# broadinstitute/Tangram

Measured on NVIDIA H100. Metric: map_cells_to_space iterations/sec, higher is better.
Workload: dtype bf16 operands / f32 accumulate+state

## Files before the change

### tangram_b200/csrc/gemm_tc.cuh

```cuda
#pragma once
#include <cuda.h>
#include <cstdio>
#include "common.cuh"
#include "gemm_simt.cuh"

namespace tgb {

constexpr int TC_BM = 128;
constexpr int TC_BK = 64;
constexpr int TC_MMA_K = 16;
constexpr int TC_BN = 256;
constexpr int TC_THREADS = 384;
constexpr int TC_ACC = TC_BN / 2;

__device__ __forceinline__ uint32_t smem_u32(const void* p) { return (uint32_t)__cvta_generic_to_shared(p); }

__device__ __forceinline__ void mbar_init(uint64_t* bar, uint32_t count) {
  asm volatile("mbarrier.init.shared::cta.b64 [%0], %1;" ::"r"(smem_u32(bar)), "r"(count));
}
__device__ __forceinline__ void mbar_expect_tx(uint64_t* bar, uint32_t bytes) {
  asm volatile("mbarrier.arrive.expect_tx.shared::cta.b64 _, [%0], %1;" ::"r"(smem_u32(bar)), "r"(bytes) : "memory");
}
__device__ __forceinline__ void mbar_wait(uint64_t* bar, uint32_t parity) {
  asm volatile(
      "{\n\t.reg .pred p;\n\t"
      "WAIT_LOOP:\n\t"
      "mbarrier.try_wait.parity.shared::cta.b64 p, [%0], %1;\n\t"
      "@p bra WAIT_DONE;\n\t"
      "bra WAIT_LOOP;\n\t"
      "WAIT_DONE:\n\t}"
      ::"r"(smem_u32(bar)), "r"(parity) : "memory");
}
__device__ __forceinline__ void mbar_arrive(uint64_t* bar) {
  asm volatile("mbarrier.arrive.shared::cta.b64 _, [%0];" ::"r"(smem_u32(bar)) : "memory");
}
__device__ __forceinline__ void fence_barrier_init() { asm volatile("fence.mbarrier_init.release.cluster;" ::: "memory"); }
__device__ __forceinline__ void mbar_arrive_cluster(uint64_t* bar, uint32_t cta) {
  asm volatile(
      "{\n\t.reg .b32 ra;\n\t"
      "mapa.shared::cluster.u32 ra, %0, %1;\n\t"
      "mbarrier.arrive.shared::cluster.b64 _, [ra];\n\t}"
      ::"r"(smem_u32(bar)), "r"(cta) : "memory");
}
__device__ __forceinline__ int cluster_rank() { uint32_t r; asm volatile("mov.u32 %0, %%cluster_ctarank;" : "=r"(r)); return (int)r; }
__device__ __forceinline__ int cluster_index() { uint32_t r; asm volatile("mov.u32 %0, %%clusterid.x;" : "=r"(r)); return (int)r; }
__device__ __forceinline__ int cluster_count() { uint32_t r; asm volatile("mov.u32 %0, %%nclusterid.x;" : "=r"(r)); return (int)r; }
__device__ __forceinline__ void cluster_sync() {
  asm volatile("barrier.cluster.arrive.release;\n\tbarrier.cluster.wait.acquire;" ::: "memory");
}

constexpr uint64_t kPolicyEvictNormal = 0x1000000000000000ull;
constexpr uint64_t kPolicyEvictLast = 0x14F0000000000000ull;
constexpr uint64_t kPolicyEvictFirst = 0x12F0000000000000ull;
__device__ __forceinline__ void prefetch_l2(const void* p) { asm volatile("prefetch.global.L2 [%0];" ::"l"(p)); }
__device__ __forceinline__ void tma_load_2d(const CUtensorMap* map, uint64_t* bar, void* dst, int c0, int c1, uint64_t policy) {
  asm volatile(
      "cp.async.bulk.tensor.2d.shared::cluster.global.tile.mbarrier::complete_tx::bytes.L2::cache_hint [%0], [%1, {%3, %4}], [%2], %5;"
      ::"r"(smem_u32(dst)), "l"(map), "r"(smem_u32(bar)), "r"(c0), "r"(c1), "l"(policy) : "memory");
}
__device__ __forceinline__ void tma_load_2d_pair(const CUtensorMap* map, uint64_t* bar, void* dst, int c0, int c1, uint64_t policy) {
  asm volatile(
      "cp.async.bulk.tensor.2d.shared::cluster.global.tile.mbarrier::complete_tx::bytes.multicast::cluster.L2::cache_hint"
      " [%0], [%1, {%3, %4}], [%2], %5, %6;"
      ::"r"(smem_u32(dst)), "l"(map), "r"(smem_u32(bar)), "r"(c0), "r"(c1), "h"((uint16_t)0x3), "l"(policy) : "memory");
}
__device__ __forceinline__ void tma_prefetch_desc(const CUtensorMap* map) {
  asm volatile("prefetch.tensormap [%0];" ::"l"(map) : "memory");
}
__device__ __forceinline__ void tma_store_2d(const CUtensorMap* map, const void* src, int c0, int c1, uint64_t policy) {
  asm volatile(
      "cp.async.bulk.tensor.2d.global.shared::cta.bulk_group.L2::cache_hint [%0, {%2, %3}], [%1], %4;"
      ::"l"(map), "r"(smem_u32(src)), "r"(c0), "r"(c1), "l"(policy) : "memory");
}
__device__ __forceinline__ void bulk_commit() { asm volatile("cp.async.bulk.commit_group;" ::: "memory"); }
__device__ __forceinline__ void bulk_wait_read_all() { asm volatile("cp.async.bulk.wait_group.read 0;" ::: "memory"); }
__device__ __forceinline__ void fence_proxy_async_smem() { asm volatile("fence.proxy.async.shared::cta;" ::: "memory"); }
template <int ID>
__device__ __forceinline__ void named_bar_sync(int threads) {
  asm volatile("bar.sync %0, %1;" ::"n"(ID), "r"(threads) : "memory");
}
__device__ __forceinline__ void ldmatrix_x4(uint32_t addr, uint32_t (&r)[4]) {
  asm volatile("ldmatrix.sync.aligned.m8n8.x4.shared.b16 {%0, %1, %2, %3}, [%4];"
               : "=r"(r[0]), "=r"(r[1]), "=r"(r[2]), "=r"(r[3]) : "r"(addr) : "memory");
}
__device__ __forceinline__ void stmatrix_x4(uint32_t addr, const uint32_t (&r)[4]) {
  asm volatile("stmatrix.sync.aligned.m8n8.x4.shared.b16 [%0], {%1, %2, %3, %4};"
               ::"r"(addr), "r"(r[0]), "r"(r[1]), "r"(r[2]), "r"(r[3]) : "memory");
}

__device__ __forceinline__ void setmaxnreg_producer() { asm volatile("setmaxnreg.dec.sync.aligned.u32 40;"); }
__device__ __forceinline__ void setmaxnreg_consumer() { asm volatile("setmaxnreg.inc.sync.aligned.u32 232;"); }

__device__ __forceinline__ void wgmma_fence() { asm volatile("wgmma.fence.sync.aligned;" ::: "memory"); }
__device__ __forceinline__ void wgmma_commit() { asm volatile("wgmma.commit_group.sync.aligned;" ::: "memory"); }
template <int N>
__device__ __forceinline__ void wgmma_wait() { asm volatile("wgmma.wait_group.sync.aligned %0;" ::"n"(N) : "memory"); }
__device__ __forceinline__ void acc_fence(float (&d)[TC_ACC]) {
// ... 24 lines not shown
        "+f"(d[40]), "+f"(d[41]), "+f"(d[42]), "+f"(d[43]), "+f"(d[44]), "+f"(d[45]), "+f"(d[46]), "+f"(d[47]),
        "+f"(d[48]), "+f"(d[49]), "+f"(d[50]), "+f"(d[51]), "+f"(d[52]), "+f"(d[53]), "+f"(d[54]), "+f"(d[55]),
        "+f"(d[56]), "+f"(d[57]), "+f"(d[58]), "+f"(d[59]), "+f"(d[60]), "+f"(d[61]), "+f"(d[62]), "+f"(d[63]),
        "+f"(d[64]), "+f"(d[65]), "+f"(d[66]), "+f"(d[67]), "+f"(d[68]), "+f"(d[69]), "+f"(d[70]), "+f"(d[71]),
        "+f"(d[72]), "+f"(d[73]), "+f"(d[74]), "+f"(d[75]), "+f"(d[76]), "+f"(d[77]), "+f"(d[78]), "+f"(d[79]),
        "+f"(d[80]), "+f"(d[81]), "+f"(d[82]), "+f"(d[83]), "+f"(d[84]), "+f"(d[85]), "+f"(d[86]), "+f"(d[87]),
        "+f"(d[88]), "+f"(d[89]), "+f"(d[90]), "+f"(d[91]), "+f"(d[92]), "+f"(d[93]), "+f"(d[94]), "+f"(d[95]),
        "+f"(d[96]), "+f"(d[97]), "+f"(d[98]), "+f"(d[99]), "+f"(d[100]), "+f"(d[101]), "+f"(d[102]), "+f"(d[103]),
        "+f"(d[104]), "+f"(d[105]), "+f"(d[106]), "+f"(d[107]), "+f"(d[108]), "+f"(d[109]), "+f"(d[110]), "+f"(d[111]),
        "+f"(d[112]), "+f"(d[113]), "+f"(d[114]), "+f"(d[115]), "+f"(d[116]), "+f"(d[117]), "+f"(d[118]), "+f"(d[119]),
        "+f"(d[120]), "+f"(d[121]), "+f"(d[122]), "+f"(d[123]), "+f"(d[124]), "+f"(d[125]), "+f"(d[126]), "+f"(d[127])
      : "l"(a_desc), "l"(b_desc), "r"(accumulate), "n"(TA), "n"(TB));
}
__device__ __forceinline__ uint64_t make_smem_desc(uint32_t saddr, uint32_t lbo_bytes, uint32_t sbo_bytes) {
  uint64_t d = 0;
  d |= (uint64_t)((saddr & 0x3FFFF) >> 4);
  d |= (uint64_t)((lbo_bytes >> 4) & 0x3FFF) << 16;
  d |= (uint64_t)((sbo_bytes >> 4) & 0x3FFF) << 32;
  d |= (uint64_t)1 << 62;
  return d;
}

template <bool KMAJOR, int ROWS>
struct OperandTile {
  static constexpr int kBytes = ROWS * TC_BK * 2;
  static __device__ __forceinline__ void load(const CUtensorMap* map, uint64_t* bar, uint8_t* dst, int mn0, int k0, uint64_t policy) {
    if (KMAJOR) {
      tma_load_2d(map, bar, dst, k0, mn0, policy);
    } else {
#pragma unroll
      for (int b = 0; b < ROWS / 64; ++b) tma_load_2d(map, bar, dst + b * 8192, mn0 + b * 64, k0, policy);
    }
  }
  static __device__ __forceinline__ void load_half_pair(const CUtensorMap* map, uint64_t* bar, uint8_t* dst, int mn0, int k0, int h,
                                                        uint64_t policy) {
    constexpr int HALF = ROWS / 2;
    if (KMAJOR) {
      tma_load_2d_pair(map, bar, dst + h * HALF * 128, k0, mn0 + h * HALF, policy);
    } else {
#pragma unroll
      for (int b = 0; b < HALF / 64; ++b)
        tma_load_2d_pair(map, bar, dst + h * HALF * 128 + b * 8192, mn0 + h * HALF + b * 64, k0, policy);
    }
  }
  static __device__ __forceinline__ uint64_t desc(uint32_t saddr, int k_step ) {
    if (KMAJOR) return make_smem_desc(saddr + k_step * (TC_MMA_K * 2), 16, 1024);
    return make_smem_desc(saddr + k_step * (TC_MMA_K * 128), 8192, 1024);
  }
};

struct EpiSmem {
  uint8_t* buf;
  uint64_t* full;
  uint64_t* free;
  uint32_t parity;
};
__device__ __forceinline__ void tile_mn(int w, int tiles_m, int tiles_n, int group_m, int& m, int& n) {
  const int per_group = group_m * tiles_n;
  const int g = w / per_group, r = w - g * per_group;
  const int rows = min(group_m, tiles_m - g * group_m);
  n = r / rows;
  m = g * group_m + (r - n * rows);
}
struct TileCoord {
  int m0, n0;
  int tile_n;
  int tiles_n;
  int split;
};

__device__ __forceinline__ float quad_sum(float v) {
  v += __shfl_xor_sync(0xffffffffu, v, 1);
  v += __shfl_xor_sync(0xffffffffu, v, 2);
  return v;
}

struct TcEpiStore {
  static constexpr int kSmemBytes = 0;
  float* C; int ldc; size_t split_stride; int M;
  int accumulate;
  __device__ __forceinline__ void prologue(const TileCoord&, int) const {}
  __device__ __forceinline__ void load(int, int, const EpiSmem&) const {}
  __device__ __forceinline__ void run(const float (&d)[TC_ACC], const TileCoord& t, int row, int lane, int, const EpiSmem&) const {
    float* base = C + (size_t)t.split * split_stride;
#pragma unroll
    for (int h = 0; h < 2; ++h) {
      const int r = row + 8 * h;
      if (r >= M) continue;
#pragma unroll
      for (int j = 0; j < TC_BN / 8; ++j) {
        const int col = t.n0 + 8 * j + 2 * (lane & 3);
        if (col < ldc) {
          float2* dst = reinterpret_cast<float2*>(base + (size_t)r * ldc + col);
          float2 v = make_float2(d[4 * j + 2 * h], d[4 * j + 2 * h + 1]);
          if (accumulate) { const float2 o = *dst; v.x += o.x; v.y += o.y; }
          *dst = v;
        }
      }
    }
  }
};

struct TcEpiDpStore {
  static constexpr int kSmemBytes = TC_BM * TC_BN * 2;
  static constexpr int kHalfBytes = kSmemBytes / 2;
  static constexpr int kBoxBytes = 64 * 128;
  CUtensorMap pt_map, dq_map;
  int ld;
  const float* center;
  float* rpart;
  int M;
  __device__ __forceinline__ int boxes(int r0, int n0) const { return r0 < M ? min(TC_BN / 64, (ld - n0) / 64) : 0; }
  __device__ __forceinline__ void prologue(const TileCoord&, int) const {}
  __device__ __forceinline__ void load(int m0, int n0, const EpiSmem& es) const {
#pragma unroll
    for (int h = 0; h < 2; ++h) {
      mbar_wait(&es.free[h], es.parity ^ 1);
      const int nb = boxes(m0 + 64 * h, n0);
      mbar_expect_tx(&es.full[h], nb * kBoxBytes);
      for (int b = 0; b < nb; ++b)
        tma_load_2d(&pt_map, &es.full[h], es.buf + h * kHalfBytes + b * kBoxBytes, n0 + 64 * b, m0 + 64 * h, kPolicyEvictFirst);
    }
  }
  __device__ __forceinline__ void run(const float (&d)[TC_ACC], const TileCoord& t, int row, int lane, int cw,
                                      const EpiSmem& es) const {
    const int r0 = t.m0 + 64 * cw;
    const int nb = boxes(r0, t.n0);
    float c[2];
#pragma unroll
// ... 66 lines not shown
      float* drow = dp + (size_t)r * ld;
      float racc = 0.f;
#pragma unroll
      for (int j = 0; j < TC_BN / 8; ++j) {
        const int col = t.n0 + 8 * j + 2 * (lane & 3);
        if (live && col < ld) {
          const __nv_bfloat162 h2 = *reinterpret_cast<const __nv_bfloat162*>(prow + col);
          const __nv_bfloat162 m2 = *reinterpret_cast<const __nv_bfloat162*>(prow + plane + col);
          const __nv_bfloat162 l2 = *reinterpret_cast<const __nv_bfloat162*>(prow + 2 * plane + col);
          const float p0 = (__low2float(l2) + __low2float(m2)) + __low2float(h2);
          const float p1 = (__high2float(l2) + __high2float(m2)) + __high2float(h2);
          const float v0 = d[4 * j + 2 * h], v1 = d[4 * j + 2 * h + 1];
          racc = fmaf(p0, v0, racc);
          racc = fmaf(p1, v1, racc);
          *reinterpret_cast<float2*>(drow + col) = make_float2(v0, v1);
        }
      }
      racc = quad_sum(racc);
      if (live && (lane & 3) == 0) rpart[(size_t)t.tile_n * M + r] = racc;
    }
  }
};

struct __align__(16) RowConst { float lse, r, h, pad; };

__device__ __forceinline__ float fast_ex2(float x) { float y; asm("ex2.approx.ftz.f32 %0, %1;" : "=f"(y) : "f"(x)); return y; }
__device__ __forceinline__ float fast_rcp(float x) { float y; asm("rcp.approx.ftz.f32 %0, %1;" : "=f"(y) : "f"(x)); return y; }
__device__ __forceinline__ float fast_sqrt(float x) { float y; asm("sqrt.approx.ftz.f32 %0, %1;" : "=f"(y) : "f"(x)); return y; }

struct TcMaps { CUtensorMap m[3]; };
__device__ __constant__ int kPairA[6] = {2, 0, 1, 1, 0, 0};
__device__ __constant__ int kPairB[6] = {0, 2, 1, 0, 1, 0};

template <bool A_KMAJOR, bool B_KMAJOR, int STAGES, class Epi>
__global__ void __launch_bounds__(TC_THREADS, 1)
k_gemm_tc(const __grid_constant__ TcMaps maps_a, const __grid_constant__ TcMaps maps_b, int n_pairs,
          int k_total, int k_per_split, int tiles_m, int tiles_n, int splits, int group_m, uint64_t policy_a,
          uint64_t policy_b, int tm_off, int k_off, const __grid_constant__ Epi epi) {
  using TileA = OperandTile<A_KMAJOR, TC_BM>;
  using TileB = OperandTile<B_KMAJOR, TC_BN>;
  constexpr int kStageBytes = TileA::kBytes + TileB::kBytes;
  constexpr int kTA = A_KMAJOR ? 0 : 1, kTB = B_KMAJOR ? 0 : 1;
  constexpr uint32_t kConsumerWarps = 8;

  extern __shared__ uint8_t smem_raw[];
  uint8_t* smem = reinterpret_cast<uint8_t*>(((uintptr_t)smem_raw + 1023) & ~(uintptr_t)1023);
  __shared__ __align__(8) uint64_t full_bar[STAGES];
  __shared__ __align__(8) uint64_t empty_bar[STAGES];
  __shared__ __align__(8) uint64_t epi_full[2], epi_free[2];

  const int wg = threadIdx.x >> 7, lane = threadIdx.x & 31;
  const int tiles_mp = (tiles_m + 1) / 2;
  const int total = tiles_mp * tiles_n * splits;
  EpiSmem es{smem + STAGES * kStageBytes, epi_full, epi_free, 0};

  if (threadIdx.x == 0) {
    tma_prefetch_desc(&maps_a.m[0]);
    tma_prefetch_desc(&maps_b.m[0]);
#pragma unroll
    for (int s = 0; s < STAGES; ++s) { mbar_init(&full_bar[s], 1); mbar_init(&empty_bar[s], 2 * kConsumerWarps); }
    if constexpr (Epi::kSmemBytes > 0) {
      for (int h = 0; h < 2; ++h) { mbar_init(&epi_full[h], 1); mbar_init(&epi_free[h], 1); }
    }
    fence_barrier_init();
  }
  cluster_sync();

  if (wg == 0) {
    setmaxnreg_producer();
    if (threadIdx.x == 0) {
      uint32_t kbg = 0;
      for (int w = cluster_index(); w < total; w += cluster_count()) {
        const int z = w / (tiles_n * tiles_mp);
        int tp_i, tn_i;
        tile_mn(w - z * tiles_n * tiles_mp, tiles_mp, tiles_n, group_m, tp_i, tn_i);
        const int tm_i = 2 * tp_i + cluster_rank();
        const bool live = tm_i < tiles_m;
        const int n0 = tn_i * TC_BN, m0 = (tm_off + tm_i) * TC_BM;
        const int k_begin = k_off + z * k_per_split;
        const int k_end = min(k_total, k_begin + k_per_split);
        const int num_kb = (k_end - k_begin + TC_BK - 1) / TC_BK;
        for (int pr = 6 - n_pairs; pr < 6; ++pr) {
          const CUtensorMap* ma = &maps_a.m[kPairA[pr]];
          const CUtensorMap* mb = &maps_b.m[kPairB[pr]];
#pragma unroll 1
          for (int kb = 0; kb < num_kb; ++kb, ++kbg) {
            const int s = kbg % STAGES;
            const uint32_t ph = (kbg / STAGES) & 1;
            mbar_wait(&empty_bar[s], ph ^ 1);
            uint8_t* sa = smem + s * kStageBytes;
            uint8_t* sb = sa + TileA::kBytes;
            mbar_expect_tx(&full_bar[s], live ? kStageBytes : TileB::kBytes);
            const int k0 = k_begin + kb * TC_BK;
            if (live) TileA::load(ma, &full_bar[s], sa, m0, k0, policy_a);
            TileB::load_half_pair(mb, &full_bar[s], sb, n0, k0, cluster_rank(), policy_b);
#ifndef TGB_SKIP_EPI
            if (Epi::kSmemBytes > 0 && live && pr == 6 - n_pairs && kb + 1 == min(STAGES, num_kb)) epi.load(m0, n0, es);
#endif
          }
        }
        if (live) es.parity ^= 1;
      }
    }
  } else {
    setmaxnreg_consumer();
    const int cw = wg - 1;
    const int ct = threadIdx.x - 128;
    const int row_in_tile = 64 * cw + 16 * ((threadIdx.x >> 5) & 3) + (lane >> 2);
    float acc[TC_ACC];
#pragma unroll
    for (int i = 0; i < TC_ACC; ++i) acc[i] = 0.f;
    uint32_t kbg = 0;
    for (int w = cluster_index(); w < total; w += cluster_count()) {
      TileCoord t;
      t.split = w / (tiles_n * tiles_mp);
      int tp_i;
      tile_mn(w - t.split * tiles_n * tiles_mp, tiles_mp, tiles_n, group_m, tp_i, t.tile_n);
      t.tiles_n = tiles_n;
      t.n0 = t.tile_n * TC_BN;
      t.m0 = (tm_off + 2 * tp_i + cluster_rank()) * TC_BM;
      const bool live = t.m0 < (tm_off + tiles_m) * TC_BM;
      const int k_begin = k_off + t.split * k_per_split;
      const int k_end = min(k_total, k_begin + k_per_split);
      const int total_kb = (k_end - k_begin + TC_BK - 1) / TC_BK * n_pairs;
#ifndef TGB_SKIP_EPI
      if (live) epi.prologue(t, ct);
#endif
      acc_fence(acc);
      for (int kb = 0; kb < total_kb; ++kb, ++kbg) {
        const int s = kbg % STAGES;
        const uint32_t ph = (kbg / STAGES) & 1;
        mbar_wait(&full_bar[s], ph);
        const uint32_t sa = smem_u32(smem + s * kStageBytes) + cw * 8192;
        const uint32_t sb = smem_u32(smem + s * kStageBytes) + TileA::kBytes;
        wgmma_fence();
#pragma unroll
        for (int k = 0; k < TC_BK / TC_MMA_K; ++k)
          wgmma_m64n256k16<kTA, kTB>(acc, TileA::desc(sa, k), TileB::desc(sb, k), (kb > 0 || k > 0) ? 1u : 0u);
        wgmma_commit();
        wgmma_wait<1>();
        if (kb > 0 && lane < 2) mbar_arrive_cluster(&empty_bar[(kbg - 1) % STAGES], lane);
      }
      wgmma_wait<0>();
      acc_fence(acc);
      if (total_kb > 0 && lane < 2) mbar_arrive_cluster(&empty_bar[(kbg - 1) % STAGES], lane);
#ifndef TGB_SKIP_EPI
      if (t.m0 < (tm_off + tiles_m) * TC_BM) {
        epi.run(acc, t, t.m0 + row_in_tile, lane, cw, es);
        es.parity ^= 1;
      }
#endif
    }
  }
  cluster_sync();
}

typedef CUresult (*PFN_encodeTiled)(CUtensorMap*, CUtensorMapDataType, cuuint32_t, void*, const cuuint64_t*,
                                    const cuuint64_t*, const cuuint32_t*, const cuuint32_t*, CUtensorMapInterleave,
                                    CUtensorMapSwizzle, CUtensorMapL2promotion, CUtensorMapFloatOOBfill);

struct TcContext {
  PFN_encodeTiled encode = nullptr;
  int num_sms = 132;
  const void* smem_fn[16] = {};
  int smem_bytes[16] = {};
  int clusters[16] = {};
};

static inline int tc_init(TcContext& tc, char* err, size_t n) {
  void* fn = nullptr;
  cudaDriverEntryPointQueryResult qres;
  cudaError_t e = cudaGetDriverEntryPoint("cuTensorMapEncodeTiled", &fn, cudaEnableDefault, &qres);
  if (e != cudaSuccess || fn == nullptr || qres != cudaDriverEntryPointSuccess) {
    snprintf(err, n, "cuTensorMapEncodeTiled not available from the driver (%s)", cudaGetErrorString(e));
    return -2;
  }
  tc.encode = (PFN_encodeTiled)fn;
  int dev = 0;
  cudaGetDevice(&dev);
  cudaDeviceGetAttribute(&tc.num_sms, cudaDevAttrMultiProcessorCount, dev);
  return 0;
}

static inline int tc_make_map(TcContext& tc, CUtensorMap* map, const void* base, uint64_t cols, uint64_t rows,
                              uint64_t ld, uint32_t box_inner, uint32_t box_outer, char* err, size_t n) {
  cuuint64_t dims[2] = {cols, rows};
  cuuint64_t strides[1] = {ld * 2};
  cuuint32_t box[2] = {box_inner, box_outer};
  cuuint32_t estr[2] = {1, 1};
  CUresult r = tc.encode(map, CU_TENSOR_MAP_DATA_TYPE_BFLOAT16, 2, const_cast<void*>(base), dims, strides, box, estr,
                         CU_TENSOR_MAP_INTERLEAVE_NONE, CU_TENSOR_MAP_SWIZZLE_128B, CU_TENSOR_MAP_L2_PROMOTION_L2_256B,
                         CU_TENSOR_MAP_FLOAT_OOB_FILL_NONE);
  if (r != CUDA_SUCCESS) {
    snprintf(err, n, "cuTensorMapEncodeTiled failed (%d) cols=%llu rows=%llu ld=%llu box=%ux%u", (int)r,
             (unsigned long long)cols, (unsigned long long)rows, (unsigned long long)ld, box_inner, box_outer);
    return -2;
  }
  return 0;
}

template <class Kern, class... Args>
static inline int tc_launch(TcContext& tc, Kern kern, int smem, long long pairs, int keep_sms, cudaStream_t s, const char* name,
                            char* err, size_t n, Args... args) {
  cudaLaunchAttribute attr[1];
  attr[0].id = cudaLaunchAttributeClusterDimension;
  attr[0].val.clusterDim.x = 2;
  attr[0].val.clusterDim.y = 1;
  attr[0].val.clusterDim.z = 1;
  cudaLaunchConfig_t cfg = {};
  cfg.blockDim = dim3(TC_THREADS);
  cfg.dynamicSmemBytes = (size_t)smem;
  cfg.stream = s;
  cfg.attrs = attr;
  cfg.numAttrs = 1;
  const void* key = reinterpret_cast<const void*>(kern);
  int slot = -1;
  for (int i = 0; i < 16; ++i) {
    if (tc.smem_fn[i] == key) { slot = i; break; }
    if (tc.smem_fn[i] == nullptr && slot < 0) slot = i;
  }
  if (slot < 0) { snprintf(err, n, "launch %s: more than 16 tensor-core kernels", name); return -2; }
  if (tc.smem_fn[slot] != key || tc.smem_bytes[slot] != smem) {
    cudaError_t e = cudaFuncSetAttribute(kern, cudaFuncAttributeMaxDynamicSharedMemorySize, smem);
    if (e != cudaSuccess) { snprintf(err, n, "cudaFuncSetAttribute(smem=%d): %s", smem, cudaGetErrorString(e)); return -2; }
    cfg.gridDim = dim3(2);
    int c = 0;
    e = cudaOccupancyMaxActiveClusters(&c, kern, &cfg);
    if (e != cudaSuccess || c < 1) {
      snprintf(err, n, "launch %s: no 2-CTA cluster with %d B of shared memory fits (%s)", name, smem, cudaGetErrorString(e));
      return -2;
    }
    tc.smem_fn[slot] = key; tc.smem_bytes[slot] = smem; tc.clusters[slot] = c;
  }
  const int clusters = std::max(1, tc.clusters[slot] - (keep_sms + 1) / 2);
  cfg.gridDim = dim3((unsigned)(2 * (pairs < clusters ? pairs : clusters)));
  cudaError_t e = cudaLaunchKernelEx(&cfg, kern, args...);
  if (e == cudaSuccess) e = cudaGetLastError();
  if (e != cudaSuccess) { snprintf(err, n, "launch %s: %s", name, cudaGetErrorString(e)); return -2; }
  return 0;
}

constexpr int TC_STAGE_BYTES = (TC_BM + TC_BN) * TC_BK * 2;
constexpr int TC_SMEM_LIMIT = 227 * 1024;
template <class Epi>
constexpr int tc_stages() {
  const int fit = (TC_SMEM_LIMIT - 2048 - Epi::kSmemBytes) / TC_STAGE_BYTES;
  return fit < 4 ? fit : 4;
}
template <class Epi>
constexpr int tc_smem() { return tc_stages<Epi>() * TC_STAGE_BYTES + Epi::kSmemBytes + 1024; }
constexpr int TC_SMEM = tc_smem<TcEpiStore>();
static inline int tc_dp_row_parts(int V) { return (int)ceil_div(V, TC_BN); }
static inline int tc_splits(int num_sms, long long tiles, long long k_total, int min_k) {
  long long s = (2LL * num_sms + tiles - 1) / tiles;
  const long long max_s = (k_total + min_k - 1) / min_k;
  if (s > max_s) s = max_s;
  if (s < 1) s = 1;
  const long long kps = ((k_total + s - 1) / s + TC_BK - 1) / TC_BK * TC_BK;
  return (int)((k_total + kps - 1) / kps);
}
static inline int tc_splits_for_chain(long long k_total, int max_chain) {
  long long s = (k_total + max_chain - 1) / max_chain;
  if (s < 1) s = 1;
  const long long kps = ((k_total + s - 1) / s + TC_BK - 1) / TC_BK * TC_BK;
  return (int)((k_total + kps - 1) / kps);
}
static inline int tc_forward_splits(int num_sms, int N, int V, int Ke) {
  return tc_splits(num_sms, (long long)ceil_div(V, TC_BM) * ceil_div(Ke, TC_BN), N, 512);
}
static inline int tc_kps(int k_total, int splits) {
  return (int)(round_up(ceil_div(k_total, splits), TC_BK));
}
static inline long long tc_pairs(int tiles_m, int tiles_n, int splits) { return (long long)(tiles_m + 1) / 2 * tiles_n * splits; }

static inline int tc_make_maps(TcContext& tc, TcMaps* maps, const __nv_bfloat16* base, size_t plane_elems, int n_planes,
                               uint64_t cols, uint64_t rows, uint64_t ld, uint32_t bi, uint32_t bo, char* err, size_t n) {
  for (int p = 0; p < 3; ++p) {
    const __nv_bfloat16* ptr = base + (size_t)(p < n_planes ? p : 0) * plane_elems;
    if (tc_make_map(tc, &maps->m[p], ptr, cols, rows, ld, bi, bo, err, n)) return -2;
  }
  return 0;
}

struct TcPlan {
  TcMaps a, b;
  CUtensorMap pt, dq;
  bool ready = false;
};

static inline int tc_forward_plan(TcContext& tc, TcPlan& pl, const __nv_bfloat16* P, size_t p_plane, const __nv_bfloat16* Sx,
                                  size_t s_plane, int planes, int N, int V, int Ke, int ld, char* err, size_t n) {
  if (tc_make_maps(tc, &pl.a, P, p_plane, planes, V, N, ld, 64, 64, err, n)) return -2;
  if (tc_make_maps(tc, &pl.b, Sx, s_plane, planes, Ke, N, Ke, 64, 64, err, n)) return -2;
  pl.ready = true;
  return 0;
}
static inline int tc_forward_launch(TcContext& tc, const TcPlan& pl, int n_pairs, float* out, int N, int V, int Ke, int splits,
                                    cudaStream_t s, char* err, size_t n) {
  auto kern = k_gemm_tc<false, false, tc_stages<TcEpiStore>(), TcEpiStore>;
  TcEpiStore epi{out, Ke, (size_t)V * Ke, V, 0};
  const int tm = (int)ceil_div(V, TC_BM), tn = (int)ceil_div(Ke, TC_BN);
  return tc_launch(tc, kern, TC_SMEM, tc_pairs(tm, tn, splits), 0, s, "tc_gemm_fwd", err, n, pl.a, pl.b, n_pairs, N, tc_kps(N, splits),
                   tm, tn, splits, 1, kPolicyEvictNormal, kPolicyEvictNormal, 0, 0, epi);
}
static inline int tc_forward_launch_rows(TcContext& tc, const TcPlan& pl, int n_pairs, float* out, int accumulate, int row0, int row1,
                                         int V, int Ke, int keep_sms, cudaStream_t s, char* err, size_t n) {
  auto kern = k_gemm_tc<false, false, tc_stages<TcEpiStore>(), TcEpiStore>;
  TcEpiStore epi{out, Ke, (size_t)V * Ke, V, accumulate};
  const int tm = (int)ceil_div(V, TC_BM), tn = (int)ceil_div(Ke, TC_BN);
  return tc_launch(tc, kern, TC_SMEM, tc_pairs(tm, tn, 1), keep_sms, s, "tc_gemm_fwd", err, n, pl.a, pl.b, n_pairs, row1,
                   (int)round_up(row1 - row0, TC_BK), tm, tn, 1, 1, kPolicyEvictNormal, kPolicyEvictNormal, 0, row0, epi);
}

static inline int tc_dpstore_plan(TcContext& tc, TcPlan& pl, const __nv_bfloat16* Sxb, size_t s_plane, const __nv_bfloat16* dYb,
                                  size_t dy_plane, int planes, int N, int V, int Ke, char* err, size_t n) {
  if (tc_make_maps(tc, &pl.a, Sxb, s_plane, planes, Ke, N, Ke, 64, TC_BM, err, n)) return -2;
  if (tc_make_maps(tc, &pl.b, dYb, dy_plane, planes, Ke, V, Ke, 64, TC_BN / 2, err, n)) return -2;
  pl.ready = true;
  return 0;
}
static inline int tc_dpstore_epi_plan(TcContext& tc, TcPlan& pl, const __nv_bfloat16* Pt, const __nv_bfloat16* dq, int N, int ld,
                                      char* err, size_t n) {
  if (tc_make_map(tc, &pl.pt, Pt, ld, N, ld, 64, 64, err, n)) return -2;
  return tc_make_map(tc, &pl.dq, dq, ld, N, ld, 64, 64, err, n);
}
template <class Epi>
static inline int tc_dpstore_launch(TcContext& tc, const TcPlan& pl, int n_pairs, const Epi& epi, int row0, int row1, int V, int Ke,
                                    int keep_sms, cudaStream_t s, char* err, size_t n) {
  const int tn = (int)ceil_div(V, TC_BN);
  auto kern = k_gemm_tc<true, true, tc_stages<Epi>(), Epi>;
  constexpr int smem = tc_smem<Epi>();
  const int tm0 = row0 / TC_BM, tm = (int)ceil_div(row1, TC_BM) - tm0;
  return tc_launch(tc, kern, smem, tc_pairs(tm, tn, 1), keep_sms, s, "tc_gemm_bwd_dp", err, n, pl.a, pl.b, n_pairs, Ke, Ke, tm, tn, 1, 1,
                   kPolicyEvictNormal, kPolicyEvictLast, tm0, 0, epi);
}

}
```

### tangram_b200/csrc/tangram_b200.cu

```cuda
#include "../../include/tangram_b200.h"

#include <algorithm>
#include <cmath>
#include <cstdarg>
#include <cstdio>
#include <cstdlib>
#include <cstring>
#include <mutex>
#include <string>
#include <thread>
#include <vector>

#include "common.cuh"
#include "kernels_elem.cuh"
#include "gemm_simt.cuh"
#include "gemm_tc.cuh"
#include "adam_rows.cuh"
#include "legacy_rng.cuh"
#include "agreement.cuh"
#include "annotate.cuh"
#include "project.cuh"
#include "group_stats.cuh"
#include "neighbors.cuh"
#include "mt19937_jump.h"
// ... 1990 lines not shown
      if (nr) CK(cudaMemcpy(out_host, d.p, nr * sizeof(float), cudaMemcpyDefault));
      if (hp.n) CK(cudaMemcpy(out_host + nr, hp.p, hp.n * sizeof(float), cudaMemcpyDefault));
    }
    return TGB200_OK;
  };
  if (nm == "Y") { src = h->Y.p; cnt = vk; }
  else if (nm == "M") return state(h->M, h->Mh);
  else if (nm == "v") return state(h->v, h->vh);
  else if (nm == "m") return h->bf16 ? state(h->mb, h->mbh) : state(h->m, h->mh);
  else if (nm == "Pb" && h->x3) return widened(h->Pb.p, nv, 3);
  else if (nm == "Pf" && !h->tcm) { src = h->Pf.p; cnt = nv; }
  else if (nm == "dpf" && h->x3) { src = h->dpf.p; cnt = nv; }
  else if (nm == "stats") { src = reinterpret_cast<const float*>(h->stats.p); cnt = (int64_t)h->N * 4; }
  else if (nm == "rowc" && h->bf16) { src = reinterpret_cast<const float*>(h->rowc.p); cnt = (int64_t)h->N * 4; }
  else if (nm == "zsum" && h->bf16) { src = h->zsum.p; cnt = h->N; }
  else if (nm == "inv_zt" && h->bf16) { src = h->inv_zt.p; cnt = h->N; }
  else if (nm == "lseA" && h->bf16) { src = h->lseA; cnt = h->N; }
  else if (nm == "lseT" && h->bf16) { src = h->lseT; cnt = h->N; }
  else if (nm == "pxsum" && h->pxsum.p) { src = h->pxsum.p; cnt = h->N; }
  else if (nm == "l1sum" && h->l1sum.p) { src = h->l1sum.p; cnt = h->N; }
  else if (nm == "l2sum" && h->l2sum.p) { src = h->l2sum.p; cnt = h->N; }
  else if (nm == "dY") {
    src = h->dY.p; cnt = vk;
    if (h->tcm && out_host) {
      if (cap < cnt) return fail(TGB200_ERR_INVALID, "buffer 'dY' needs %lld floats", (long long)cnt);
      CKS(widen_bf16(h->dYb.p, vk, h->x3 ? 3 : 1, out_host));
      *n = cnt;
      return TGB200_OK;
    }
  }
  else if ((nm == "dq" || nm == "Pb") && h->bf16) return widened(nm == "dq" ? h->dq.p : h->Pb.p, nv, 1);
  else if (nm == "rcenter" && h->bf16) { src = h->rcenter.p; cnt = h->N; }
  else if (nm == "rdot") { src = h->rdot.p; cnt = h->N; }
  else if (nm == "ngc") { src = h->ngc.p; cnt = h->K; }
  else if (nm == "ngr") { src = h->ngr.p; cnt = h->V; }
  else if (nm == "nwg" && h->nwg.p) { src = h->nwg.p; cnt = h->K; }
  else if (nm == "nag" && h->nag.p) { src = h->nag.p; cnt = h->K; }
  else if (nm == "Sx") { src = h->Sx.p; cnt = (int64_t)h->N * h->Ke; }
  else if (nm == "tail") { src = h->Y.p + vk; cnt = kTail; }
  else if (h->constrained && (nm == "F" || nm == "f" || nm == "mF" || nm == "vF")) {
    src = nm == "F" ? h->Fl.p : nm == "f" ? h->fsig.p : nm == "mF" ? h->mF.p : h->vF.p;
    cnt = h->N;
  }
  else if (nm == "Sf" && h->constrained) { src = h->Sf.p; cnt = (int64_t)h->N * h->Ke; }
  else if (nm == "fscal" && h->constrained) { src = h->fscal.p; cnt = 2; }
  else if (nm == "shape") {
    *n = 5;
    if (!out_host) return TGB200_OK;
    if (cap < 5) return fail(TGB200_ERR_INVALID, "cap < 5");
    out_host[0] = (float)h->Ke; out_host[1] = (float)h->ld; out_host[2] = (float)h->fwd_splits; out_host[3] = (float)h->r_parts;
    out_host[4] = (float)h->nchunks;
    return TGB200_OK;
  } else if (nm == "ring") {
    *n = 1;
    if (!out_host) return TGB200_OK;
    if (cap < 1) return fail(TGB200_ERR_INVALID, "cap < 1");
    out_host[0] = (float)h->ring_rows;
    return TGB200_OK;
  } else if (nm == "legacy_init") {
    *n = 8;
    if (!out_host) return TGB200_OK;
    if (cap < 8) return fail(TGB200_ERR_INVALID, "cap < 8");
    for (int i = 0; i < 8; ++i) out_host[i] = h->legacy_stats[i];
    return TGB200_OK;
  } else return fail(TGB200_ERR_INVALID, "unknown debug buffer '%s'", name);
  *n = cnt;
// ... 674 lines not shown
}

extern "C" int tgb200_group_stats(const float* X, int64_t x_ld, const int64_t* indptr, const int32_t* indices,
                                  const float* data, int64_t nnz, int64_t rows, int64_t n_genes,
                                  const int32_t* labels, int32_t n_labels, double* sum_out, double* sumsq_out,
                                  int64_t* nnz_out, int64_t block_rows, int32_t device, void* stream) {
  return group_stats_pass(GsValue::kIdentity, 1.0, X, x_ld, indptr, indices, data, nnz, rows, n_genes, labels, n_labels,
                          sum_out, sumsq_out, nnz_out, block_rows, device, stream);
}

extern "C" int tgb200_group_stats_expm1(const float* X, int64_t x_ld, const int64_t* indptr, const int32_t* indices,
                                        const float* data, int64_t nnz, int64_t rows, int64_t n_genes,
                                        const int32_t* labels, int32_t n_labels, double* sum_out, double* sumsq_out,
                                        int64_t* nnz_out, int64_t block_rows, int32_t device, void* stream,
                                        double scale) {
  if (!std::isfinite(scale)) return fail(TGB200_ERR_INVALID, "scale=%g is not finite", scale);
  return group_stats_pass(GsValue::kExpm1, scale, X, x_ld, indptr, indices, data, nnz, rows, n_genes, labels, n_labels,
                          sum_out, sumsq_out, nnz_out, block_rows, device, stream);
}

#ifdef TGB_OVERLAP_PROBE
extern "C" TGB200_API int tgb200_debug_overlap_probe(tgb200_mapper* h, int32_t kind, int32_t cap, int32_t update_ctas,
                                                     int32_t what, int32_t reps, float* out) {
  if (!h || !out || reps < 1 || what < 1 || what > 3) return fail(TGB200_ERR_INVALID, "bad argument");
  if (!h->bf16 || !h->pipelined || h->host_state || !h->plan_dp.ready || !h->plan_fwd.ready)
    return fail(TGB200_ERR_STATE, "needs a resident, pipelined bf16 handle that has run an iteration");
  CK(cudaSetDevice(h->cfg.device));
  const int c0 = h->chunk_row[0], c1 = h->chunk_row[1], c2 = h->chunk_row[2];
  const AdamScalars a = adam_scalars(h->cfg, h->step > 0 ? h->step : 1, 0.1f);
  const AdamRowsArgs ar{h->M.p, h->mb.p, h->v.p, h->dq.p, h->Pb.p, reinterpret_cast<const RowConst*>(h->rowc.p),
                        h->zsum.p, h->pxsum.p, h->l1sum.p, h->l2sum.p, h->ld, h->V, c0, c1,
                        h->cfg.lambda_r, h->cfg.lambda_l1, h->cfg.lambda_l2, a};
  const bool plain = ar.lam_r == 0.f && ar.lam_l1 == 0.f && ar.lam_l2 == 0.f;
  const int keep = cap > 0 ? std::max(0, h->tc.num_sms - 2 * cap) : 0;
  cudaEvent_t ev[4];
  for (auto& e : ev) CK(cudaEventCreate(&e));
  int st = TGB200_OK;
  CK(cudaDeviceSynchronize());
  for (int r = 0; r < reps && st == TGB200_OK; ++r) {
    CK(cudaEventRecord(ev[0], h->hi));
    CK(cudaStreamWaitEvent(h->lo, ev[0], 0));
    if (what & 1) {
      if (kind == 0) {
        TcEpiDpStore epi{h->plan_dp.pt, h->plan_dp.dq, h->ld, h->rcenter.p, h->rpart.p, h->N};
        st = tc_dpstore_launch(h->tc, h->plan_dp, 1, epi, c1, c2, h->V, h->Ke, keep, h->hi, g_err, sizeof(g_err));
      } else {
        st = tc_forward_launch_rows(h->tc, h->plan_fwd, 1, h->Y.p, 1, c1, c2, h->V, h->Ke, keep, h->hi, g_err, sizeof(g_err));
      }
    }
    if (what & 2) {
      if (update_ctas <= 0) {
        if (adam_rows_launch(ar, h->lo)) st = fail(TGB200_ERR_CUDA, "launch adam_rows");
      } else if (plain) {
        k_adam_rows_probe<true><<<update_ctas, 512, 0, h->lo>>>(ar);
      } else {
        k_adam_rows_probe<false><<<update_ctas, 512, 0, h->lo>>>(ar);
      }
      if (cudaGetLastError() != cudaSuccess) st = fail(TGB200_ERR_CUDA, "launch adam_rows_probe");
    }
    CK(cudaEventRecord(ev[1], h->hi));
    CK(cudaEventRecord(ev[2], h->lo));
    CK(cudaStreamWaitEvent(h->hi, ev[2], 0));
    CK(cudaEventRecord(ev[3], h->hi));
    CK(cudaEventSynchronize(ev[3]));
    for (int i = 0; i < 3; ++i) CK(cudaEventElapsedTime(&out[3 * r + i], ev[0], ev[i + 1]));
  }
  for (auto& e : ev) cudaEventDestroy(e);
// ... 205 lines not shown
```

Before: 48.81.

## Template GEMM cluster size for 4-CTA multicast and batch epilogue accumulate loads

Makes the TMA multicast cluster size a template parameter, so B tiles can be shared across 2 or 4 CTAs, chosen through the TGB200_CLUSTER environment variable (default 2). The store epilogue now issues L2 prefetches for the accumulate target in the prologue and batches eight float2 loads before the stores to raise memory-level parallelism. By default only the epilogue batching and prefetch change behavior. The 4-CTA path adds scheduling constraints and tail waste.

```diff
diff --git a/tangram_b200/csrc/gemm_tc.cuh b/tangram_b200/csrc/gemm_tc.cuh
--- a/tangram_b200/csrc/gemm_tc.cuh
+++ b/tangram_b200/csrc/gemm_tc.cuh
@@ -1,6 +1,7 @@
 #pragma once
 #include <cuda.h>
 #include <cstdio>
+#include <cstdlib>
 #include "common.cuh"
 #include "gemm_simt.cuh"
 
@@ -58,11 +59,12 @@
       "cp.async.bulk.tensor.2d.shared::cluster.global.tile.mbarrier::complete_tx::bytes.L2::cache_hint [%0], [%1, {%3, %4}], [%2], %5;"
       ::"r"(smem_u32(dst)), "l"(map), "r"(smem_u32(bar)), "r"(c0), "r"(c1), "l"(policy) : "memory");
 }
-__device__ __forceinline__ void tma_load_2d_pair(const CUtensorMap* map, uint64_t* bar, void* dst, int c0, int c1, uint64_t policy) {
+template <int CL>
+__device__ __forceinline__ void tma_load_2d_mc(const CUtensorMap* map, uint64_t* bar, void* dst, int c0, int c1, uint64_t policy) {
   asm volatile(
       "cp.async.bulk.tensor.2d.shared::cluster.global.tile.mbarrier::complete_tx::bytes.multicast::cluster.L2::cache_hint"
       " [%0], [%1, {%3, %4}], [%2], %5, %6;"
-      ::"r"(smem_u32(dst)), "l"(map), "r"(smem_u32(bar)), "r"(c0), "r"(c1), "h"((uint16_t)0x3), "l"(policy) : "memory");
+      ::"r"(smem_u32(dst)), "l"(map), "r"(smem_u32(bar)), "r"(c0), "r"(c1), "h"((uint16_t)((1u << CL) - 1)), "l"(policy) : "memory");
 }
 __device__ __forceinline__ void tma_prefetch_desc(const CUtensorMap* map) {
   asm volatile("prefetch.tensormap [%0];" ::"l"(map) : "memory");
@@ -153,15 +155,17 @@
       for (int b = 0; b < ROWS / 64; ++b) tma_load_2d(map, bar, dst + b * 8192, mn0 + b * 64, k0, policy);
     }
   }
-  static __device__ __forceinline__ void load_half_pair(const CUtensorMap* map, uint64_t* bar, uint8_t* dst, int mn0, int k0, int h,
-                                                        uint64_t policy) {
-    constexpr int HALF = ROWS / 2;
+  template <int CL>
+  static __device__ __forceinline__ void load_part(const CUtensorMap* map, uint64_t* bar, uint8_t* dst, int mn0, int k0, int p,
+                                                   uint64_t policy) {
+    constexpr int PART = ROWS / CL;
+    static_assert(PART % 64 == 0, "a part is whole 64-row boxes");
     if (KMAJOR) {
-      tma_load_2d_pair(map, bar, dst + h * HALF * 128, k0, mn0 + h * HALF, policy);
+      tma_load_2d_mc<CL>(map, bar, dst + p * PART * 128, k0, mn0 + p * PART, policy);
     } else {
 #pragma unroll
-      for (int b = 0; b < HALF / 64; ++b)
-        tma_load_2d_pair(map, bar, dst + h * HALF * 128 + b * 8192, mn0 + h * HALF + b * 64, k0, policy);
+      for (int b = 0; b < PART / 64; ++b)
+        tma_load_2d_mc<CL>(map, bar, dst + p * PART * 128 + b * 8192, mn0 + p * PART + b * 64, k0, policy);
     }
   }
   static __device__ __forceinline__ uint64_t desc(uint32_t saddr, int k_step ) {
@@ -200,22 +204,39 @@
   static constexpr int kSmemBytes = 0;
   float* C; int ldc; size_t split_stride; int M;
   int accumulate;
-  __device__ __forceinline__ void prologue(const TileCoord&, int) const {}
+  __device__ __forceinline__ void prologue(const TileCoord& t, int ct) const {
+    if (!accumulate) return;
+    const float* base = C + (size_t)t.split * split_stride;
+    for (int i = ct; i < TC_BM * (TC_BN / 32); i += 256) {
+      const int row = t.m0 + i / (TC_BN / 32), col = t.n0 + (i % (TC_BN / 32)) * 32;
+      if (row < M && col < ldc) prefetch_l2(base + (size_t)row * ldc + col);
+    }
+  }
   __device__ __forceinline__ void load(int, int, const EpiSmem&) const {}
+  static constexpr int kBatch = 8;
   __device__ __forceinline__ void run(const float (&d)[TC_ACC], const TileCoord& t, int row, int lane, int, const EpiSmem&) const {
     float* base = C + (size_t)t.split * split_stride;
 #pragma unroll
     for (int h = 0; h < 2; ++h) {
       const int r = row + 8 * h;
       if (r >= M) continue;
-#pragma unroll
-      for (int j = 0; j < TC_BN / 8; ++j) {
-        const int col = t.n0 + 8 * j + 2 * (lane & 3);
-        if (col < ldc) {
-          float2* dst = reinterpret_cast<float2*>(base + (size_t)r * ldc + col);
-          float2 v = make_float2(d[4 * j + 2 * h], d[4 * j + 2 * h + 1]);
-          if (accumulate) { const float2 o = *dst; v.x += o.x; v.y += o.y; }
-          *dst = v;
+      float* crow = base + (size_t)r * ldc;
+#pragma unroll
+      for (int j0 = 0; j0 < TC_BN / 8; j0 += kBatch) {
+        float2 o[kBatch];
+#pragma unroll
+        for (int j = 0; j < kBatch; ++j) {
+          const int col = t.n0 + 8 * (j0 + j) + 2 * (lane & 3);
+          o[j] = accumulate && col < ldc ? *reinterpret_cast<const float2*>(crow + col) : make_float2(0.f, 0.f);
+        }
+#pragma unroll
+        for (int j = 0; j < kBatch; ++j) {
+          const int col = t.n0 + 8 * (j0 + j) + 2 * (lane & 3);
+          if (col < ldc) {
+            float2 v = make_float2(d[4 * (j0 + j) + 2 * h], d[4 * (j0 + j) + 2 * h + 1]);
+            if (accumulate) { v.x += o[j].x; v.y += o[j].y; }
+            *reinterpret_cast<float2*>(crow + col) = v;
+          }
         }
       }
     }
@@ -348,7 +369,7 @@
 __device__ __constant__ int kPairA[6] = {2, 0, 1, 1, 0, 0};
 __device__ __constant__ int kPairB[6] = {0, 2, 1, 0, 1, 0};
 
-template <bool A_KMAJOR, bool B_KMAJOR, int STAGES, class Epi>
+template <bool A_KMAJOR, bool B_KMAJOR, int STAGES, int CL, class Epi>
 __global__ void __launch_bounds__(TC_THREADS, 1)
 k_gemm_tc(const __grid_constant__ TcMaps maps_a, const __grid_constant__ TcMaps maps_b, int n_pairs,
           int k_total, int k_per_split, int tiles_m, int tiles_n, int splits, int group_m, uint64_t policy_a,
@@ -366,7 +387,7 @@
   __shared__ __align__(8) uint64_t epi_full[2], epi_free[2];
 
   const int wg = threadIdx.x >> 7, lane = threadIdx.x & 31;
-  const int tiles_mp = (tiles_m + 1) / 2;
+  const int tiles_mp = (tiles_m + CL - 1) / CL;
   const int total = tiles_mp * tiles_n * splits;
   EpiSmem es{smem + STAGES * kStageBytes, epi_full, epi_free, 0};
 
@@ -374,7 +395,7 @@
     tma_prefetch_desc(&maps_a.m[0]);
     tma_prefetch_desc(&maps_b.m[0]);
 #pragma unroll
-    for (int s = 0; s < STAGES; ++s) { mbar_init(&full_bar[s], 1); mbar_init(&empty_bar[s], 2 * kConsumerWarps); }
+    for (int s = 0; s < STAGES; ++s) { mbar_init(&full_bar[s], 1); mbar_init(&empty_bar[s], CL * kConsumerWarps); }
     if constexpr (Epi::kSmemBytes > 0) {
       for (int h = 0; h < 2; ++h) { mbar_init(&epi_full[h], 1); mbar_init(&epi_free[h], 1); }
     }
@@ -390,7 +411,7 @@
         const int z = w / (tiles_n * tiles_mp);
         int tp_i, tn_i;
         tile_mn(w - z * tiles_n * tiles_mp, tiles_mp, tiles_n, group_m, tp_i, tn_i);
-        const int tm_i = 2 * tp_i + cluster_rank();
+        const int tm_i = CL * tp_i + cluster_rank();
         const bool live = tm_i < tiles_m;
         const int n0 = tn_i * TC_BN, m0 = (tm_off + tm_i) * TC_BM;
         const int k_begin = k_off + z * k_per_split;
@@ -409,7 +430,7 @@
             mbar_expect_tx(&full_bar[s], live ? kStageBytes : TileB::kBytes);
             const int k0 = k_begin + kb * TC_BK;
             if (live) TileA::load(ma, &full_bar[s], sa, m0, k0, policy_a);
-            TileB::load_half_pair(mb, &full_bar[s], sb, n0, k0, cluster_rank(), policy_b);
+            TileB::template load_part<CL>(mb, &full_bar[s], sb, n0, k0, cluster_rank(), policy_b);
 #ifndef TGB_SKIP_EPI
             if (Epi::kSmemBytes > 0 && live && pr == 6 - n_pairs && kb + 1 == min(STAGES, num_kb)) epi.load(m0, n0, es);
 #endif
@@ -434,7 +455,7 @@
       tile_mn(w - t.split * tiles_n * tiles_mp, tiles_mp, tiles_n, group_m, tp_i, t.tile_n);
       t.tiles_n = tiles_n;
       t.n0 = t.tile_n * TC_BN;
-      t.m0 = (tm_off + 2 * tp_i + cluster_rank()) * TC_BM;
+      t.m0 = (tm_off + CL * tp_i + cluster_rank()) * TC_BM;
       const bool live = t.m0 < (tm_off + tiles_m) * TC_BM;
       const int k_begin = k_off + t.split * k_per_split;
       const int k_end = min(k_total, k_begin + k_per_split);
@@ -455,11 +476,11 @@
           wgmma_m64n256k16<kTA, kTB>(acc, TileA::desc(sa, k), TileB::desc(sb, k), (kb > 0 || k > 0) ? 1u : 0u);
         wgmma_commit();
         wgmma_wait<1>();
-        if (kb > 0 && lane < 2) mbar_arrive_cluster(&empty_bar[(kbg - 1) % STAGES], lane);
+        if (kb > 0 && lane < CL) mbar_arrive_cluster(&empty_bar[(kbg - 1) % STAGES], lane);
       }
       wgmma_wait<0>();
       acc_fence(acc);
-      if (total_kb > 0 && lane < 2) mbar_arrive_cluster(&empty_bar[(kbg - 1) % STAGES], lane);
+      if (total_kb > 0 && lane < CL) mbar_arrive_cluster(&empty_bar[(kbg - 1) % STAGES], lane);
 #ifndef TGB_SKIP_EPI
       if (t.m0 < (tm_off + tiles_m) * TC_BM) {
         epi.run(acc, t, t.m0 + row_in_tile, lane, cw, es);
@@ -481,6 +502,7 @@
   const void* smem_fn[16] = {};
   int smem_bytes[16] = {};
   int clusters[16] = {};
+  int cluster = 2;
 };
 
 static inline int tc_init(TcContext& tc, char* err, size_t n) {
@@ -495,6 +517,11 @@
   int dev = 0;
   cudaGetDevice(&dev);
   cudaDeviceGetAttribute(&tc.num_sms, cudaDevAttrMultiProcessorCount, dev);
+  if (const char* e = getenv("TGB200_CLUSTER")) {
+    const int c = atoi(e);
+    if (c != 2 && c != 4) { snprintf(err, n, "TGB200_CLUSTER=%s: expected 2 or 4", e); return -1; }
+    tc.cluster = c;
+  }
   return 0;
 }
 
@@ -515,12 +542,12 @@
   return 0;
 }
 
-template <class Kern, class... Args>
-static inline int tc_launch(TcContext& tc, Kern kern, int smem, long long pairs, int keep_sms, cudaStream_t s, const char* name,
+template <int CL, class Kern, class... Args>
+static inline int tc_launch(TcContext& tc, Kern kern, int smem, long long items, int keep_sms, cudaStream_t s, const char* name,
                             char* err, size_t n, Args... args) {
   cudaLaunchAttribute attr[1];
   attr[0].id = cudaLaunchAttributeClusterDimension;
-  attr[0].val.clusterDim.x = 2;
+  attr[0].val.clusterDim.x = CL;
   attr[0].val.clusterDim.y = 1;
   attr[0].val.clusterDim.z = 1;
   cudaLaunchConfig_t cfg = {};
@@ -539,17 +566,17 @@
   if (tc.smem_fn[slot] != key || tc.smem_bytes[slot] != smem) {
     cudaError_t e = cudaFuncSetAttribute(kern, cudaFuncAttributeMaxDynamicSharedMemorySize, smem);
     if (e != cudaSuccess) { snprintf(err, n, "cudaFuncSetAttribute(smem=%d): %s", smem, cudaGetErrorString(e)); return -2; }
-    cfg.gridDim = dim3(2);
+    cfg.gridDim = dim3(CL);
     int c = 0;
     e = cudaOccupancyMaxActiveClusters(&c, kern, &cfg);
     if (e != cudaSuccess || c < 1) {
-      snprintf(err, n, "launch %s: no 2-CTA cluster with %d B of shared memory fits (%s)", name, smem, cudaGetErrorString(e));
+      snprintf(err, n, "launch %s: no %d-CTA cluster with %d B of shared memory fits (%s)", name, CL, smem, cudaGetErrorString(e));
       return -2;
     }
     tc.smem_fn[slot] = key; tc.smem_bytes[slot] = smem; tc.clusters[slot] = c;
   }
-  const int clusters = std::max(1, tc.clusters[slot] - (keep_sms + 1) / 2);
-  cfg.gridDim = dim3((unsigned)(2 * (pairs < clusters ? pairs : clusters)));
+  const int clusters = std::max(1, tc.clusters[slot] - (keep_sms + CL - 1) / CL);
+  cfg.gridDim = dim3((unsigned)(CL * (items < clusters ? items : clusters)));
   cudaError_t e = cudaLaunchKernelEx(&cfg, kern, args...);
   if (e == cudaSuccess) e = cudaGetLastError();
   if (e != cudaSuccess) { snprintf(err, n, "launch %s: %s", name, cudaGetErrorString(e)); return -2; }
@@ -587,7 +614,9 @@
 static inline int tc_kps(int k_total, int splits) {
   return (int)(round_up(ceil_div(k_total, splits), TC_BK));
 }
-static inline long long tc_pairs(int tiles_m, int tiles_n, int splits) { return (long long)(tiles_m + 1) / 2 * tiles_n * splits; }
+static inline long long tc_items(int tiles_m, int tiles_n, int splits, int cl) {
+  return (long long)(tiles_m + cl - 1) / cl * tiles_n * splits;
+}
 
 static inline int tc_make_maps(TcContext& tc, TcMaps* maps, const __nv_bfloat16* base, size_t plane_elems, int n_planes,
                                uint64_t cols, uint64_t rows, uint64_t ld, uint32_t bi, uint32_t bo, char* err, size_t n) {
@@ -600,6 +629,7 @@
 
 struct TcPlan {
   TcMaps a, b;
+  TcMaps bq;
   CUtensorMap pt, dq;
   bool ready = false;
 };
@@ -611,27 +641,31 @@
   pl.ready = true;
   return 0;
 }
+static inline int tc_forward_go(TcContext& tc, const TcPlan& pl, int n_pairs, const TcEpiStore& epi, int k_total, int kps, int splits,
+                                int k_off, int V, int Ke, int keep_sms, cudaStream_t s, char* err, size_t n) {
+  const int tm = (int)ceil_div(V, TC_BM), tn = (int)ceil_div(Ke, TC_BN);
+  constexpr int st = tc_stages<TcEpiStore>();
+  if (tc.cluster == 4)
+    return tc_launch<4>(tc, k_gemm_tc<false, false, st, 4, TcEpiStore>, TC_SMEM, tc_items(tm, tn, splits, 4), keep_sms, s, "tc_gemm_fwd",
+                        err, n, pl.a, pl.b, n_pairs, k_total, kps, tm, tn, splits, 1, kPolicyEvictNormal, kPolicyEvictNormal, 0, k_off, epi);
+  return tc_launch<2>(tc, k_gemm_tc<false, false, st, 2, TcEpiStore>, TC_SMEM, tc_items(tm, tn, splits, 2), keep_sms, s, "tc_gemm_fwd",
+                      err, n, pl.a, pl.b, n_pairs, k_total, kps, tm, tn, splits, 1, kPolicyEvictNormal, kPolicyEvictNormal, 0, k_off, epi);
+}
 static inline int tc_forward_launch(TcContext& tc, const TcPlan& pl, int n_pairs, float* out, int N, int V, int Ke, int splits,
                                     cudaStream_t s, char* err, size_t n) {
-  auto kern = k_gemm_tc<false, false, tc_stages<TcEpiStore>(), TcEpiStore>;
-  TcEpiStore epi{out, Ke, (size_t)V * Ke, V, 0};
-  const int tm = (int)ceil_div(V, TC_BM), tn = (int)ceil_div(Ke, TC_BN);
-  return tc_launch(tc, kern, TC_SMEM, tc_pairs(tm, tn, splits), 0, s, "tc_gemm_fwd", err, n, pl.a, pl.b, n_pairs, N, tc_kps(N, splits),
-                   tm, tn, splits, 1, kPolicyEvictNormal, kPolicyEvictNormal, 0, 0, epi);
+  return tc_forward_go(tc, pl, n_pairs, TcEpiStore{out, Ke, (size_t)V * Ke, V, 0}, N, tc_kps(N, splits), splits, 0, V, Ke, 0, s, err, n);
 }
 static inline int tc_forward_launch_rows(TcContext& tc, const TcPlan& pl, int n_pairs, float* out, int accumulate, int row0, int row1,
                                          int V, int Ke, int keep_sms, cudaStream_t s, char* err, size_t n) {
-  auto kern = k_gemm_tc<false, false, tc_stages<TcEpiStore>(), TcEpiStore>;
-  TcEpiStore epi{out, Ke, (size_t)V * Ke, V, accumulate};
-  const int tm = (int)ceil_div(V, TC_BM), tn = (int)ceil_div(Ke, TC_BN);
-  return tc_launch(tc, kern, TC_SMEM, tc_pairs(tm, tn, 1), keep_sms, s, "tc_gemm_fwd", err, n, pl.a, pl.b, n_pairs, row1,
-                   (int)round_up(row1 - row0, TC_BK), tm, tn, 1, 1, kPolicyEvictNormal, kPolicyEvictNormal, 0, row0, epi);
+  return tc_forward_go(tc, pl, n_pairs, TcEpiStore{out, Ke, (size_t)V * Ke, V, accumulate}, row1, (int)round_up(row1 - row0, TC_BK), 1,
+                       row0, V, Ke, keep_sms, s, err, n);
 }
 
 static inline int tc_dpstore_plan(TcContext& tc, TcPlan& pl, const __nv_bfloat16* Sxb, size_t s_plane, const __nv_bfloat16* dYb,
                                   size_t dy_plane, int planes, int N, int V, int Ke, char* err, size_t n) {
   if (tc_make_maps(tc, &pl.a, Sxb, s_plane, planes, Ke, N, Ke, 64, TC_BM, err, n)) return -2;
   if (tc_make_maps(tc, &pl.b, dYb, dy_plane, planes, Ke, V, Ke, 64, TC_BN / 2, err, n)) return -2;
+  if (tc_make_maps(tc, &pl.bq, dYb, dy_plane, planes, Ke, V, Ke, 64, TC_BN / 4, err, n)) return -2;
   pl.ready = true;
   return 0;
 }
@@ -644,11 +678,13 @@
 static inline int tc_dpstore_launch(TcContext& tc, const TcPlan& pl, int n_pairs, const Epi& epi, int row0, int row1, int V, int Ke,
                                     int keep_sms, cudaStream_t s, char* err, size_t n) {
   const int tn = (int)ceil_div(V, TC_BN);
-  auto kern = k_gemm_tc<true, true, tc_stages<Epi>(), Epi>;
-  constexpr int smem = tc_smem<Epi>();
+  constexpr int st = tc_stages<Epi>(), smem = tc_smem<Epi>();
   const int tm0 = row0 / TC_BM, tm = (int)ceil_div(row1, TC_BM) - tm0;
-  return tc_launch(tc, kern, smem, tc_pairs(tm, tn, 1), keep_sms, s, "tc_gemm_bwd_dp", err, n, pl.a, pl.b, n_pairs, Ke, Ke, tm, tn, 1, 1,
-                   kPolicyEvictNormal, kPolicyEvictLast, tm0, 0, epi);
-}
-
-}
+  if (tc.cluster == 4)
+    return tc_launch<4>(tc, k_gemm_tc<true, true, st, 4, Epi>, smem, tc_items(tm, tn, 1, 4), keep_sms, s, "tc_gemm_bwd_dp", err, n, pl.a,
+                        pl.bq, n_pairs, Ke, Ke, tm, tn, 1, 1, kPolicyEvictNormal, kPolicyEvictLast, tm0, 0, epi);
+  return tc_launch<2>(tc, k_gemm_tc<true, true, st, 2, Epi>, smem, tc_items(tm, tn, 1, 2), keep_sms, s, "tc_gemm_bwd_dp", err, n, pl.a,
+                      pl.b, n_pairs, Ke, Ke, tm, tn, 1, 1, kPolicyEvictNormal, kPolicyEvictLast, tm0, 0, epi);
+}
+
+}
diff --git a/tangram_b200/csrc/tangram_b200.cu b/tangram_b200/csrc/tangram_b200.cu
--- a/tangram_b200/csrc/tangram_b200.cu
+++ b/tangram_b200/csrc/tangram_b200.cu
@@ -2046,6 +2046,7 @@
   else if ((nm == "dq" || nm == "Pb") && h->bf16) return widened(nm == "dq" ? h->dq.p : h->Pb.p, nv, 1);
   else if (nm == "rcenter" && h->bf16) { src = h->rcenter.p; cnt = h->N; }
   else if (nm == "rdot") { src = h->rdot.p; cnt = h->N; }
+  else if (nm == "rpart") { src = h->rpart.p; cnt = (int64_t)h->r_parts * h->N; }
   else if (nm == "ngc") { src = h->ngc.p; cnt = h->K; }
   else if (nm == "ngr") { src = h->ngr.p; cnt = h->V; }
   else if (nm == "nwg" && h->nwg.p) { src = h->nwg.p; cnt = h->K; }
@@ -2786,7 +2787,7 @@
                         h->zsum.p, h->pxsum.p, h->l1sum.p, h->l2sum.p, h->ld, h->V, c0, c1,
                         h->cfg.lambda_r, h->cfg.lambda_l1, h->cfg.lambda_l2, a};
   const bool plain = ar.lam_r == 0.f && ar.lam_l1 == 0.f && ar.lam_l2 == 0.f;
-  const int keep = cap > 0 ? std::max(0, h->tc.num_sms - 2 * cap) : 0;
+  const int keep = cap > 0 ? std::max(0, h->tc.num_sms - h->tc.cluster * cap) : 0;
   cudaEvent_t ev[4];
   for (auto& e : ev) CK(cudaEventCreate(&e));
   int st = TGB200_OK;
```

Measured after the change: 49.59 (median of 6 runs). 1.6% higher.
